# ColumbiaDVMM/ColumbiaImageSearch

Measured on AMD Instinct MI355X. Metric: queries/sec @ recall@10 on 10M LOPQ index, higher is better.
Workload: dtype f64

## Files before the change

### columbiaimagesearch_amd/csrc/lopq_scan3.hip

```cpp
#include "scan_common.h"
#include <cmath>
#include <cstdio>
#include <cstdlib>

typedef unsigned short u16x2_t __attribute__((ext_vector_type(2)));

static __device__ __forceinline__ uint32_t pk_add_u16(uint32_t a, uint32_t b) {
    return __builtin_bit_cast(uint32_t, (u16x2_t)(__builtin_bit_cast(u16x2_t, a) + __builtin_bit_cast(u16x2_t, b)));
}
static __device__ __forceinline__ uint32_t pk_subsat_u16(uint32_t a, uint32_t b) {
    return __builtin_bit_cast(uint32_t, __builtin_elementwise_sub_sat(__builtin_bit_cast(u16x2_t, a), __builtin_bit_cast(u16x2_t, b)));
}

static __device__ __forceinline__ uint32_t pk_min_u16(uint32_t a, uint32_t b) {
    return __builtin_bit_cast(uint32_t, __builtin_elementwise_min(__builtin_bit_cast(u16x2_t, a), __builtin_bit_cast(u16x2_t, b)));
}

static const int S3G = 4;

#ifdef CIS_S3_COUNTERS
__device__ unsigned long long g_s3_ctr[16];
#define S3_CLK() ((long long)__builtin_amdgcn_s_memtime())
#define S3_CTR(i, v) do { if (threadIdx.x == 0) atomicAdd(&g_s3_ctr[i], (unsigned long long)(v)); } while (0)
extern "C" int cis_debug_counters3(unsigned long long* out, int reset) {
// ... 140 lines not shown
    for (int r = 0; r < NR; ++r) {
        const bool kp = keep[r] && s[r] <= cut;
        const unsigned long long m = __ballot(kp);
        const int idx = ncnt + __builtin_amdgcn_mbcnt_hi((unsigned)(m >> 32), __builtin_amdgcn_mbcnt_lo((unsigned)m, 0));
        if (kp) rk[idx] = ent[r];
        ncnt += __popcll(m);
    }
    __builtin_amdgcn_fence(__ATOMIC_RELEASE, "wavefront");
    __builtin_amdgcn_wave_barrier();
    return ncnt;
}

template <int M, int NR, int NW>
__device__ __forceinline__ int wave_compact3_exact(uint32_t* rk, int cnt, int L, int Lw, const QScale& qs, Scan3Shared* sh, int w,
                                                   const uint8_t* __restrict__ codes, int64_t start, int K,
                                                   const double* __restrict__ t0, const double* __restrict__ t1, uint32_t& dup_pos) {
    const int lane = threadIdx.x & 63;
    const uint64_t INF64 = 0x7ff0000000000000ull;
    uint32_t hi[NR], lo[NR], ent[NR];
    bool keep[NR];
    uint32_t mn = 0xffffffffu, mx = 0u;
#pragma unroll
    for (int r = 0; r < NR; ++r) {
        const int e = r * 64 + lane;
        keep[r] = e < cnt;
        ent[r] = keep[r] ? rk[e] : 0xffffffffu;
        hi[r] = 0xffffffffu;
        lo[r] = 0xffffffffu;
    }
#pragma unroll
    for (int r = 0; r < NR; ++r) {
        if (r * 64 >= cnt) break;
        const CodeWords<M> cw = load_code<M>(codes, start + (keep[r] ? (ent[r] & 0xffffu) : 0u));
        const uint64_t k = keep[r] ? (uint64_t)__double_as_longlong(adc64_words<M>(cw.w, K, t0, t1)) : ~0ull;
        hi[r] = (uint32_t)(k >> 32);
        lo[r] = (uint32_t)k;
        mn = (keep[r] && hi[r] < mn) ? hi[r] : mn;
        mx = (keep[r] && hi[r] > mx) ? hi[r] : mx;
    }
    wave_minmax_step<1>(mn, mx); wave_minmax_step<2>(mn, mx); wave_minmax_step<4>(mn, mx);
    wave_minmax_step<8>(mn, mx); wave_minmax_step<16>(mn, mx); wave_minmax_step<32>(mn, mx);
    mn = (uint32_t)__builtin_amdgcn_readfirstlane((int)mn);
    mx = (uint32_t)__builtin_amdgcn_readfirstlane((int)mx);
    uint32_t vhiL = mx;
    uint64_t boundL = INF64;
    if (cnt >= L) {
        const uint32_t vhi = wave_kth_bisect<NR>(hi, keep, mn, mx, L);
        vhiL = vhi;
        boundL = hi_to_bound(vhi);
        int c_less = 0, g = 0;
#pragma unroll
        for (int r = 0; r < NR; ++r) {
            c_less += __popcll(__ballot(keep[r] && hi[r] < vhi));
// ... 125 lines not shown
    for (int i = 1; i < OCT; ++i) {
        a0 = pk_add_u16(a0, f[i][0]);
        a1 = pk_add_u16(a1, f[i][1]);
    }
    u32x2_t r;
    r[0] = a0; r[1] = a1;
    return r;
}

static __device__ __forceinline__ uint32_t ld16(const uint16_t* p) { return *reinterpret_cast<const volatile uint16_t*>(p); }
static __device__ __forceinline__ void st16(uint16_t* p, uint32_t v) { *reinterpret_cast<volatile uint16_t*>(p) = (uint16_t)v; }

template <int M, int NR, int U, int NW>
__device__ __forceinline__ void scan3_group(const WorkItem* __restrict__ items, const TabDesc* __restrict__ tabs,
                                            const int (&item_idx)[S3G], int ng,
                                            const double* __restrict__ T, const float* __restrict__ T32,
                                            const uint8_t* __restrict__ codes, int K, int L, int S,
                                            uint64_t* __restrict__ item_surv, int* __restrict__ item_n, float* __restrict__ item_slack,
                                            unsigned long long* __restrict__ qbound, char* smem, bool two_pass) {
    constexpr int G = S3G;
    constexpr int R = NR * 64 - 8;
    constexpr int nf = M / 2;
    constexpr int OCT = M >= 8 ? 8 : 4, NU = M / OCT;
    constexpr uint32_t CAP = 65535u / M;
    char* tab = smem;
    uint32_t* rk_all = reinterpret_cast<uint32_t*>(smem + (size_t)K * M * G * 2);
    Scan3Shared* sh = reinterpret_cast<Scan3Shared*>(rk_all + G * NW * R);
    uint16_t* thr1 = reinterpret_cast<uint16_t*>(sh + G);
    const int tid = threadIdx.x, lane = tid & 63;
    const int w = __builtin_amdgcn_readfirstlane(tid >> 6);
    const long long c0 = S3_CLK();
// ... 418 lines not shown
                        u0 = u;
                        continue;
                    }
                    const int idx = cnt[g] + __builtin_amdgcn_mbcnt_hi((unsigned)(m >> 32), __builtin_amdgcn_mbcnt_lo((unsigned)m, 0));
                    if ((m >> lane) & 1ull) rk[idx] = entry(u);
                    cnt[g] += n;
                    u0 = u + 1;
                }
                if (!full) break;
                const QScale qsg = load_scale(&sh[g]);
                int c2 = wave_compact3<M, NR, NW>(rk, cnt[g], L, Lw, R - 64, qsg, &sh[g], w);
                if (c2 < 0) {
                    uint32_t dp = 0xffffffffu;
                    const WorkItem itg = items[item_idx[g]];
                    c2 = wave_compact3_exact<M, NR, NW>(rk, cnt[g], L, Lw, qsg, &sh[g], w, codes, start, K,
                                                        T + (int64_t)itg.tab0 * nf * K, T + (int64_t)itg.tab1 * nf * K, dp);
                    dp = (uint32_t)__builtin_amdgcn_readfirstlane((int)dp);
                    if (dp != 0xffffffffu) {
                        dup[g] = load_code<M>(codes, start + (int64_t)dp);
                        has_dup[g] = true;
                        any_dup = true;
                    }
                }
                cnt[g] = c2;
                const uint32_t thg = lds_ld(&sh[g].thr);
                if (lane == 0) st16(&thr1[g], thg + 1u);
                const unsigned long long dup_on = has_dup[g] ? ~0ull : 0ull;
#pragma unroll
                for (int u = 0; u < U; ++u) {
                    const uint32_t sg = (g & 1) ? (d[u][g >> 1] >> 16) : (d[u][g >> 1] & 0xffffu);
                    bool same = true;
// ... 40 lines not shown
        }
        uint64_t* out = item_surv + (int64_t)item_idx[g] * S + off;
        for (int e = lane; e < cnt[g]; e += 64) {
            const uint32_t x = rk[e];
            out[e] = ((uint64_t)(x >> 16) << 32) | (x & 0xffffu);
        }
        if (tid == 0) item_n[item_idx[g]] = total;
    }
    S3_CTR(7, S3_CLK() - c0);
    S3_CTR(0, 1);
}

template <int M, int NR, int U, int NW, int WPE>
__global__ __launch_bounds__(NW * 64) __attribute__((amdgpu_waves_per_eu(WPE, WPE))) void k_adc_scan3(
    const WorkItem* __restrict__ items, const TabDesc* __restrict__ tabs, const int* __restrict__ slots,
    const int* __restrict__ n_slots_ptr, const double* __restrict__ T, const float* __restrict__ T32,
    const uint8_t* __restrict__ codes, int K, int L, int S, int* __restrict__ queue_ctr ,
    uint64_t* __restrict__ item_surv, int* __restrict__ item_n, float* __restrict__ item_slack,
    unsigned long long* __restrict__ qbound , int two_pass, int single_queue ) {
    extern __shared__ __attribute__((aligned(16))) char smem[];
    constexpr int G = S3G;
    constexpr int R = NR * 64 - 8;
    int* s_next = reinterpret_cast<int*>(smem + (size_t)K * M * G * 2 + (size_t)G * NW * R * 4 + G * sizeof(Scan3Shared) + 32);
    const int* qs = n_slots_ptr + 8;
    const int home = blockIdx.x & 7;
    const long long k0 = S3_CLK();
    (void)k0;
    for (int a = 0; a < 8; ++a) {
        const int x = (home + a) & 7;
        const int qstart = qs[x];
        const int count = single_queue ? (x == 0 ? qs[1] - qstart : 0) : qs[x + 1] - qstart;
// ... 27 lines not shown
                } else {
                    idx[g] = idx[0];
                }
            }
            if (!same) {
                for (int g2 = 0; g2 < ng; ++g2) {
                    int oi[G];
#pragma unroll
                    for (int g = 0; g < G; ++g) {
                        oi[g] = idx[0];
#pragma unroll
                        for (int gg = 1; gg < G; ++gg)
                            if (gg == g2) oi[g] = idx[gg];
                    }
                    if (g2 > 0) __syncthreads();
                    scan3_group<M, NR, U, NW>(items, tabs, oi, 1, T, T32, codes, K, L, S, item_surv, item_n, item_slack, qbound, smem, two_pass != 0);
                }
                continue;
            }
            scan3_group<M, NR, U, NW>(items, tabs, idx, ng, T, T32, codes, K, L, S, item_surv, item_n, item_slack, qbound, smem, two_pass != 0);
        }
    }
    S3_CTR(9, S3_CLK() - k0);
    S3_CTR(10, 1);
}

struct Slot4 {
    int item[S3G], tab0[S3G], tab1[S3G], q[S3G];
    float qinv[S3G];
    int start_lo, start_hi, len, ng;
    int ist_lo[S3G], ist_hi[S3G], ilen[S3G];
};
struct Scan4Shared {
    double inv_up, ub;
    uint64_t ext;
// ... 1294 lines not shown
                       S5_B, nsamp, ss_env, hits, hitn, slack, cnt_ok, ovf);
    hipLaunchKernelGGL(k_scan5_tau<S5_B / 64>, dim3((unsigned)((nq + 3) / 4)), dim3(256), 0, st, bmin, S5_B, nsamp, plan, nq, P, tau);
    if (ev_main) (void)hipEventRecord(ev_main, st);
    hipLaunchKernelGGL((k_adc_scan5<M, false, WPE>), dim3(grid), dim3(256), lds, st, items, tabs, slots, n_slots, T32, T, codes, K, g.S, tau, bmin, S5_B, nsamp,
                       ss_env, hits, hitn, slack, cnt_ok, ovf);
    const int64_t max_slots = n_items + 8;
    hipLaunchKernelGGL(k_scan5_check, dim3((unsigned)((max_slots + 255) / 256)), dim3(256), 0, st, slots, n_slots, items, plan, cnt_ok, ovf, L, fhdr, fslots, hitn,
                       qctr + 9);
    if (getenv("CIS_SCAN5_DEBUG")) {
        int h[6] = {0, 0, 0, 0, 0, 0};
        if (hipMemcpyAsync(h, qctr + 9, sizeof(h), hipMemcpyDeviceToHost, st) == hipSuccess && hipStreamSynchronize(st) == hipSuccess)
            fprintf(stderr, "[cis] k_adc_scan5: %d slots to the fall-back list\n", h[1]);
    }
    constexpr int U = 4, NW = 4;
    constexpr int WPE3 = 4;
    hipLaunchKernelGGL((k_adc_scan3<M, NR, U, NW, WPE3>), dim3(256), dim3(NW * 64), g.lds, st, items, tabs, fslots, fhdr + 8, T, T32, codes, K, L, g.S, fhdr, hits, hitn,
                       slack, qbound, g.long_chunks ? 0 : 1, 1);
}

void launch_scan5(int M, const Scan3Geom& g, int64_t n_items, int nq, hipStream_t st, const WorkItem* items, const TabDesc* tabs, const int* slots,
                  const int* n_slots, const PlanOut* plan, const double* T, const float* T32, const uint8_t* codes, int K, int L, int* qctr, uint64_t* hits,
                  int* hitn, float* slack, unsigned long long* qbound, int* fhdr, int* fslots, void* ws, hipEvent_t ev_main) {
    if (M == 4) {
        if (L <= 184) launch_scan5_t<4, 4>(g, n_items, nq, st, items, tabs, slots, n_slots, plan, T, T32, codes, K, L, qctr, hits, hitn, slack, qbound, fhdr, fslots, ws, ev_main);
        else launch_scan5_t<4, 8>(g, n_items, nq, st, items, tabs, slots, n_slots, plan, T, T32, codes, K, L, qctr, hits, hitn, slack, qbound, fhdr, fslots, ws, ev_main);
    } else {
        if (L <= 184) launch_scan5_t<8, 4>(g, n_items, nq, st, items, tabs, slots, n_slots, plan, T, T32, codes, K, L, qctr, hits, hitn, slack, qbound, fhdr, fslots, ws, ev_main);
        else launch_scan5_t<8, 8>(g, n_items, nq, st, items, tabs, slots, n_slots, plan, T, T32, codes, K, L, qctr, hits, hitn, slack, qbound, fhdr, fslots, ws, ev_main);
    }
}

bool scan3_supported(int M, int K, int L) {
// ... 12 lines not shown
    g.long_chunks = avg_chunk >= 6144 ? 1 : 0;
    static const int s4_m16 = getenv("CIS_S4_M16") ? atoi(getenv("CIS_S4_M16")) : 1;
    if (g.two_pass == 0 && g.long_chunks && (M <= 8 || s4_m16) && L <= 128) g.two_pass = 2;
    if (const char* e = getenv("CIS_SCAN3_TWOPASS")) g.two_pass = atoi(e);
    if (force_two_pass >= 0) g.two_pass = force_two_pass;
    if (g.two_pass == 2 && M > 8 && !s4_m16 && force_two_pass != 2) g.two_pass = g.long_chunks ? 0 : 1;
    if (g.two_pass == 1 && g.long_chunks && force_two_pass < 0) g.two_pass = 0;
    if (g.two_pass < 0 || g.two_pass > 2) g.two_pass = 0;
    g.S = g.NW * (NR * 64 - 8);
    g.lds = (size_t)K * M * g.G * 2 + (size_t)g.G * g.NW * (NR * 64 - 8) * 4 + g.G * sizeof(Scan3Shared) + 32 + 16;
    return g;
}

template <int M, int NR, int NW>
static void launch_scan3_t(const Scan3Geom& g, int64_t n_items, hipStream_t st, const WorkItem* items, const TabDesc* tabs,
                           const int* slots, const int* n_slots, const double* T, const float* T32, const uint8_t* codes, int K,
                           int L, int* qctr, uint64_t* hits, int* hitn, float* slack, unsigned long long* qbound, int* fhdr, int* fslots) {
    constexpr int U = 4;
    constexpr int WPE = M == 16 ? (NW == 4 ? 3 : 2) : (NW == 4 ? 4 : (NW == 2 ? 3 : 2));
    const int by_lds = (int)(163840 / g.lds), by_waves = (WPE * 4) / NW;
    const int per_cu = by_lds < by_waves ? by_lds : by_waves;
    const int64_t resident = 256 * (per_cu < 1 ? 1 : per_cu);
    const int64_t want = (n_items + g.G - 1) / g.G + 8;
    const unsigned grid = (unsigned)(want < resident ? ((want + 7) / 8) * 8 : resident);
    if constexpr (NW == 4) {
        if (g.two_pass == 2) {
            const float z_short = getenv("CIS_S4_ZS") ? (float)atof(getenv("CIS_S4_ZS")) : CIS_S4_Z;
            const float z_long = getenv("CIS_S4_ZL") ? (float)atof(getenv("CIS_S4_ZL")) : 4.5f;
            const int frac_long = getenv("CIS_S4_FRAC") ? atoi(getenv("CIS_S4_FRAC")) : 8;
            const int nsx_long = getenv("CIS_S4_NSX") ? atoi(getenv("CIS_S4_NSX")) : 128;
            const int dyn_long = getenv("CIS_S4_DYN") ? atoi(getenv("CIS_S4_DYN")) : 0;
// ... 25 lines not shown
                    const size_t lds4 = scan4_lds(M, K, S4_LCAP_LONG, 8);
                    hipLaunchKernelGGL((k_adc_scan4<M, CIS_S4_UL, 8, WPE8, S4_LCAP_LONG>), dim3(grid_of(lds4, WPE8, 8)), dim3(8 * 64), lds4, st, items, tabs, slots,
                                       n_slots, T32, T, codes, K, L, g.S, dbg4, fhdr, fslots, hits, hitn, slack, qbound, z_long, frac_long, nsx_long, dyn_long, g.sat);
                } else {
                    const size_t lds4 = scan4_lds(M, K, S4_LCAP_LONG, NW);
                    hipLaunchKernelGGL((k_adc_scan4<M, CIS_S4_UL, NW, WPE4, S4_LCAP_LONG>), dim3(grid_of(lds4, WPE4, NW)), dim3(NW * 64), lds4, st, items, tabs, slots,
                                       n_slots, T32, T, codes, K, L, g.S, dbg4, fhdr, fslots, hits, hitn, slack, qbound, z_long, frac_long, nsx_long, dyn_long, g.sat);
                }
            }
            if (getenv("CIS_SCAN4_DEBUG")) {
                int h[6] = {0, 0, 0, 0, 0, 0};
                if (hipMemcpyAsync(h, qctr + 9, sizeof(h), hipMemcpyDeviceToHost, st) == hipSuccess && hipStreamSynchronize(st) == hipSuccess)
                    fprintf(stderr, "[cis] k_adc_scan4: %d slots, %d to the fall-back list (lists: %d overflowed, %d failed the verification, %d crowds at the cut; %d slots with items of different chunks)\n",
                            h[0], h[1], h[2], h[3], h[4], h[5]);
            }
            hipLaunchKernelGGL((k_adc_scan3<M, NR, U, NW, WPE>), dim3(256), dim3(NW * 64), g.lds, st, items, tabs, fslots, fhdr + 8, T, T32,
                               codes, K, L, g.S, fhdr, hits, hitn, slack, qbound, g.long_chunks ? 0 : 1, 1);
            return;
        }
    }
    hipLaunchKernelGGL((k_adc_scan3<M, NR, U, NW, WPE>), dim3(grid), dim3(NW * 64), g.lds, st, items, tabs, slots, n_slots, T, T32,
                       codes, K, L, g.S, qctr, hits, hitn, slack, qbound, g.two_pass, 0);
}

void launch_scan3(int M, const Scan3Geom& g, int64_t n_items, hipStream_t st, const WorkItem* items, const TabDesc* tabs,
                  const int* slots, const int* n_slots, const double* T, const float* T32, const uint8_t* codes, int K, int L,
                  int* qctr, uint64_t* hits, int* hitn, float* slack, unsigned long long* qbound, int* fhdr, int* fslots) {
#define CIS_S3_NW(MM, RR) launch_scan3_t<MM, RR, 4>(g, n_items, st, items, tabs, slots, n_slots, T, T32, codes, K, L, qctr, hits, hitn, slack, qbound, fhdr, fslots)
#define CIS_S3(MM)                   \
    do {                             \
        if (L <= 184) CIS_S3_NW(MM, 4); \
        else CIS_S3_NW(MM, 8);       \
    } while (0)
    if (M == 4) CIS_S3(4);
    else if (M == 8) CIS_S3(8);
    else CIS_S3(16);
#undef CIS_S3
#undef CIS_S3_NW
}
```

### columbiaimagesearch_amd/csrc/lopq_search.hip

```cpp
#include <atomic>
#include <chrono>
#include <mutex>
#include <algorithm>

#include "lopq_index.h"
#include "scan_common.h"


static __device__ __forceinline__ uint64_t f2bits(double d) { return (uint64_t)__double_as_longlong(d); }
static __device__ __forceinline__ uint64_t f2bits(float f) { return (uint64_t)__float_as_uint(f); }

static const int GRP_SUB = 32;
#define GRP_WORDS(V) (6 * (V) * GRP_SUB + 2)
#define GRP_TILES(V) ((2 * (V) * GRP_SUB + 1023) / 1024)

template <typename CT>
__global__ void k_rank(const CT* __restrict__ dist , int nq, int V,
                       uint16_t* __restrict__ order , CT* __restrict__ sorted ,
                       int* __restrict__ grp ) {
    extern __shared__ __attribute__((aligned(16))) char smem[];
    uint64_t* sb = reinterpret_cast<uint64_t*>(smem);
    const int q = blockIdx.x, s = blockIdx.y;
    if (q == 0 && s == 0)
        for (int i = threadIdx.x; i < 4 * V * GRP_SUB; i += blockDim.x) grp[i] = 0;
// ... 1309 lines not shown
#endif
    if (threadIdx.x < nt) ssplit[threadIdx.x] = tabs[t0 + threadIdx.x].split;
    __syncthreads();
    const bool on = k < K;
    double sc[W];
    const double* src = subs + ((int64_t)(z * nf + j) * K + (on ? k : 0)) * W;
#pragma unroll
    for (int i = 0; i < W; ++i) sc[i] = src[i];
    for (int t = 0; t < nt; ++t) {
        if (ssplit[t] != z) continue;
#ifndef CIS_TABLES_SCALAR_PX
        const double* f = sf[t];
#else
        const double* f = px + (int64_t)(t0 + t) * h + j * W;
#endif
        auto elem = [&](int i) -> double { const double df = f[i] - sc[i]; return df * df; };
        const double v = pw_leaf<double>(elem, 0, W);
        const float v32 = (float)v;
        if (on) {
#ifndef CIS_TABLES_NO_NT
            __builtin_nontemporal_store(v, &T[((int64_t)(t0 + t) * nf + j) * K + k]);
#else
            T[((int64_t)(t0 + t) * nf + j) * K + k] = v;
#endif
            if (T32) T32[((int64_t)(t0 + t) * nf + j) * K + k] = v32;
        }
        uint32_t b = on ? __float_as_uint(v32) : 0u, dummy = 0u;
        wave_minmax_step<1>(dummy, b); wave_minmax_step<2>(dummy, b); wave_minmax_step<4>(dummy, b);
        wave_minmax_step<8>(dummy, b); wave_minmax_step<16>(dummy, b); wave_minmax_step<32>(dummy, b);
        if ((threadIdx.x & 63) == 0) atomicMax(reinterpret_cast<unsigned int*>(&tabs[t0 + t].pad), b);
    }
}

__global__ void k_tables_f32(const double* __restrict__ T, int64_t n, int nf, int K, float* __restrict__ T32, TabDesc* __restrict__ tabs) {
    const int64_t e = (int64_t)blockIdx.x * blockDim.x + threadIdx.x;
    if (e >= n) return;
    const float v = (float)T[e];
    T32[e] = v;
// ... 1188 lines not shown
                if (gt == asc) { ka[i] = a1; kb[i] = b1; ka[p] = a0; kb[p] = b0; }
            }
            wave_lds_sync();
        }
    }
}

template <int CAPM, int MT , int NEMAX >
#ifndef CIS_MERGE_WPE
#define CIS_MERGE_WPE 4
#endif
__global__ __launch_bounds__(256) __attribute__((amdgpu_waves_per_eu((MT == 16 || MT == 0) ? 2 : CIS_MERGE_WPE, 8)))
void k_merge_survivors(const uint64_t* __restrict__ surv ,
                                                         const int* __restrict__ item_n, const int64_t* __restrict__ item_off,
                                                         const WorkItem* __restrict__ items, const double* __restrict__ T,
                                                         const uint8_t* __restrict__ codes, const int64_t* __restrict__ ids,
                                                         int nq, int M, int K, int limit, int S,
                                                         cis_hit* __restrict__ out_hits, int64_t* __restrict__ out_ids,
                                                         double* __restrict__ out_dists, int* __restrict__ out_n,
                                                         int32_t* __restrict__ out_cells, uint32_t* __restrict__ out_pos,
                                                         const PlanOut* __restrict__ plan, int32_t* __restrict__ out_visited,
                                                         const float* __restrict__ item_slack ) {
    extern __shared__ __attribute__((aligned(16))) char smem[];
    const int lane = threadIdx.x & 63, wq = threadIdx.x >> 6;
    const int q = blockIdx.x * 4 + wq;
    if (q >= nq) return;
    if (lane == 0 && out_visited) out_visited[q] = plan[q].visited;
    uint64_t* ka = reinterpret_cast<uint64_t*>(smem) + (size_t)wq * 2 * CAPM;
    uint64_t* kb = ka + CAPM;
    const int64_t first = item_off[q];
// ... 69 lines not shown
                if (item_slack) {
                    const float s_i = li[i] == 0 ? sl[0] : (li[i] == 1 ? sl[1] : (li[i] == 2 ? sl[2] : sl[3]));
                    keep[i] = valid[i] && ((double)__uint_as_float(hi[i]) - (double)s_i <= (double)vub);
                }
                const unsigned long long m = __ballot(keep[i]);
                idx[i] = kept + __builtin_amdgcn_mbcnt_hi((unsigned)(m >> 32), __builtin_amdgcn_mbcnt_lo((unsigned)m, 0));
                kept += __popcll(m);
            }
            if (kept > CAPM) return false;
            WorkItem its[4];
#pragma unroll
            for (int i = 0; i < 4; ++i) its[i] = items[first + (i < n_lists ? i : 0)];
#pragma unroll
            for (int i0 = 0; i0 < NE; i0 += 4) {
                int64_t startv[4];
                const double* t0v[4];
                const double* t1v[4];
                uint32_t rankv[4], pos0v[4];
#pragma unroll
                for (int i = 0; i < 4; ++i) {
                    WorkItem it = its[0];
#pragma unroll
                    for (int j = 1; j < 4; ++j)
                        if (li[i0 + i] == j) it = its[j];
                    startv[i] = it.start; rankv[i] = (uint32_t)it.rank; pos0v[i] = (uint32_t)it.pos0;
                    t0v[i] = T + (int64_t)it.tab0 * nf * K;
                    t1v[i] = T + (int64_t)it.tab1 * nf * K;
                }
                CodeWords<MT> cw[4];
#pragma unroll
                for (int i = 0; i < 4; ++i) cw[i] = load_code<MT>(codes, startv[i] + (keep[i0 + i] ? pp[i0 + i] : 0u));
                double dd[4];
#pragma unroll
                for (int i = 0; i < 4; ++i) dd[i] = adc64_words<MT>(cw[i].w, K, t0v[i], t1v[i]);
#pragma unroll
                for (int i = 0; i < 4; ++i) {
                    if (keep[i0 + i]) {
                        ka[idx[i0 + i]] = (uint64_t)__double_as_longlong(dd[i]);
                        kb[idx[i0 + i]] = ((uint64_t)rankv[i] << 32) | (uint32_t)(pos0v[i] + pp[i0 + i]);
                    }
                }
            }
            int ns = 64;
            while (ns < kept) ns <<= 1;
            for (int x = kept + lane; x < ns; x += 64) { ka[x] = ~0ull; kb[x] = ~0ull; }
            wave_lds_sync();
            wave_bitonic_lds(ka, kb, ns);
            total = kept;
            return true;
// ... 24 lines not shown
                    }
                } else {
                    for (int x0 = 0; x0 < take; x0 += 256) {
                        uint32_t p[4];
                        bool on[4];
#pragma unroll
                        for (int i = 0; i < 4; ++i) {
                            const int x = x0 + i * 64 + lane;
                            on[i] = x < take;
                            p[i] = on[i] ? (uint32_t)src[x] : 0u;
                        }
                        CodeWords<MT> cw[4];
#pragma unroll
                        for (int i = 0; i < 4; ++i) cw[i] = load_code<MT>(codes, it.start + p[i]);
                        double dd[4];
#pragma unroll
                        for (int i = 0; i < 4; ++i) dd[i] = adc64_words<MT>(cw[i].w, K, t0, t1);
#pragma unroll
                        for (int i = 0; i < 4; ++i) {
                            const int x = x0 + i * 64 + lane;
                            if (on[i]) {
                                ka[n + x] = (uint64_t)__double_as_longlong(dd[i]);
                                kb[n + x] = ((uint64_t)(uint32_t)it.rank << 32) | (uint32_t)(it.pos0 + (int)p[i]);
                            }
                        }
                    }
                }
            }
            n += take;
            total += take;
            room -= take;
            e += take;
// ... 1850 lines not shown
    TabDesc* tabs = ix->w_tabs.as<TabDesc>();
    CIS_TRY(ix->w_tord.reserve((size_t)(n_tabs + 1) * sizeof(int)));
    int* tab_order = ix->w_tord.as<int>();
    double* T = ix->w_T.as<double>();
    static const bool no_t32 = getenv("CIS_NO_T32") != nullptr && atoi(getenv("CIS_NO_T32")) != 0;
    const bool drop_t32 = no_t32 && !direct_elig && (m->w == 4 || m->w == 8 || m->w == 16 || m->w == 32) && K <= 256;
    if (!drop_t32) CIS_TRY(ix->w_T32.reserve(direct_elig ? (size_t)(n_tabs + 1) * h * sizeof(float) : (size_t)(n_tabs + 1) * nf * K * sizeof(float)));
    float* T32 = drop_t32 ? nullptr : ix->w_T32.as<float>();
    const size_t tab_lds = (size_t)(2 * h + (h < 256 ? 256 : 0)) * sizeof(double);
    const bool split_tables = (m->w == 4 || m->w == 8 || m->w == 16 || m->w == 32) && K <= 256;
    double* px_buf = nullptr;
    if (split_tables) {
        CIS_TRY(ix->w_px.reserve((size_t)(n_tabs + 1) * h * sizeof(double)));
        px_buf = ix->w_px.as<double>();
    }
    if (ct == CIS_F32) {
        if (par_plan)
            hipLaunchKernelGGL((k_plan_par<float, true>), dim3(nq), dim3(256), 0, st, ix->w_sorted.as<float>(), ix->w_order.as<uint16_t>(),
                               ix->gcount_ptr(), ix->loff_ptr(), nq, V, quota, seg_max, plan, item_off, tab_off, items,
                               tabs, nullptr, grp_base, grp_cur, tab_order, vis_list, plan_fb, vis_cap, nullptr, 0);
        hipLaunchKernelGGL((k_plan<float, true>), dim3(nq), dim3(64), plan_lds, st, ix->w_sorted.as<float>(),
                           ix->w_order.as<uint16_t>(), ix->gcount_ptr(), ix->loff_ptr(), nq, V, quota,
                           seg_max, plan, item_off, tab_off, items, tabs, nullptr, grp_base, grp_cur, tab_order, plan_fb);
        if (n_tabs > 0)
            launch_tables<float>(n_tabs, tab_lds, st, (const float*)xc, m->d_Cs32, m->d_Rt, m->d_mus, m->d_subs, tabs, tab_order, V, h,
                                 m->w, nf, K, D, T, m->prog_w, px_buf, d_tot, direct_elig ? T32 : nullptr);
    } else {
        if (par_plan)
            hipLaunchKernelGGL((k_plan_par<double, true>), dim3(nq), dim3(256), 0, st, ix->w_sorted.as<double>(), ix->w_order.as<uint16_t>(),
                               ix->gcount_ptr(), ix->loff_ptr(), nq, V, quota, seg_max, plan, item_off, tab_off, items,
                               tabs, nullptr, grp_base, grp_cur, tab_order, vis_list, plan_fb, vis_cap, nullptr, 0);
        hipLaunchKernelGGL((k_plan<double, true>), dim3(nq), dim3(64), plan_lds, st, ix->w_sorted.as<double>(),
                           ix->w_order.as<uint16_t>(), ix->gcount_ptr(), ix->loff_ptr(), nq, V, quota,
                           seg_max, plan, item_off, tab_off, items, tabs, nullptr, grp_base, grp_cur, tab_order, plan_fb);
        if (n_tabs > 0)
            launch_tables<double>(n_tabs, tab_lds, st, (const double*)xc, m->d_Cs64, m->d_Rt, m->d_mus, m->d_subs, tabs, tab_order, V,
                                  h, m->w, nf, K, D, T, m->prog_w, px_buf, d_tot, direct_elig ? T32 : nullptr);
    }
    const bool direct = direct_elig;
    if (direct) {
    } else if (split_tables && n_tabs > 0) {
        const bool few = n_tabs <= 1024;
        dim3 g((unsigned)ceil_div(n_tabs, few ? 8 : 64), (unsigned)nf, 2);
#define CIS_TFP(WW)                                                                                                                                      \
        if (few) hipLaunchKernelGGL((k_tables_from_px<WW, 8>), g, dim3(256), 0, st, px_buf, tabs, (int)n_tabs, m->d_subs, h, nf, K, T, T32, d_tot);      \
        else hipLaunchKernelGGL((k_tables_from_px<WW, 64>), g, dim3(256), 0, st, px_buf, tabs, (int)n_tabs, m->d_subs, h, nf, K, T, T32, d_tot)
        switch (m->w) {
            case 4: CIS_TFP(4); break;
            case 8: CIS_TFP(8); break;
            case 16: CIS_TFP(16); break;
            default: CIS_TFP(32); break;
        }
#undef CIS_TFP
    } else if (fast && n_tabs > 0) {
        const int64_t ne = n_tabs * nf * K;
        hipLaunchKernelGGL(k_tables_f32, dim3((unsigned)ceil_div(ne, 256)), dim3(256), 0, st, T, ne, nf, K, T32, tabs);
    }
    if (stream) {
        CIS_TRY(mark(2));
        const uint8_t* codes = ix->codes_ptr();
        const int64_t* ids = ix->ids_ptr();
// ... 219 lines not shown
            hipLaunchKernelGGL(k_copy_visited, dim3((unsigned)ceil_div(nq, 256)), dim3(256), 0, st, plan, nq, out.visited);
        CIS_CHECK_HIP(hipGetLastError());
        CIS_TRY(mark(4));
        if (ix->profiling) ix->prof.push_back(pr);
        return CIS_OK;
    }
    CIS_TRY(mark(2));
    if (n_items > 0) {
        pr.has_scan = true;
        const uint8_t* codes = ix->codes_ptr();
        const int64_t* ids = ix->ids_ptr();
        cis_hit* hits = ix->w_hits.as<cis_hit>();
        int* hitn = ix->w_hitn.as<int>();
        if (fast) {
            const bool sort_items = ix->ncells <= 65536;
            static const int env_s5 = getenv("CIS_SCAN5") ? atoi(getenv("CIS_SCAN5")) : 0;
            const bool use5 = use3 && geom3.two_pass == 2 && scan5_supported(M, K, L) && (ix->force_scan5 || (env_s5 != 0 && !ix->force_scan3 && L <= 128));
            const int G = use5 ? 8 : (use3 ? geom3.G : geom.G);
            int64_t CH = use3 ? ceil_div(ix->max_cell > 0 ? ix->max_cell : 1, (int64_t)seg_max) : 1;
            CH = CH < 1 ? 1 : (CH > 16 ? 16 : CH);
            const int64_t nkeys = 2 * ix->ncells * CH;
            const int64_t max_slots = sort_items ? (n_items + nkeys) / G + nkeys + 2 : n_items;
            CIS_TRY(ix->w_order2.reserve((size_t)(64 + 2 * nkeys + 2 * max_slots * G) * sizeof(int)));
            int* qctr = ix->w_order2.as<int>();
            int* n_slots = qctr + 8;
            int* qstart = qctr + 16;
            int* fhdr = qctr + 32;
            int* cell_cnt = qctr + 64;
            int* slot_off = cell_cnt + nkeys;
            int* slots = slot_off + nkeys;
            int* fslots = slots + max_slots * G;
            if (sort_items) {
// ... 9 lines not shown
                CIS_CHECK_HIP(hipMemsetAsync(qctr, 0, 64 * sizeof(int), st));
                hipLaunchKernelGGL(k_identity_slots, dim3((unsigned)ceil_div(n_items < 9 ? 9 : n_items, 256)), dim3(256), 0, st, n_items, G,
                                   slots, n_slots, qstart);
            }
            CIS_TRY(mark(5));
            ix->last_scan_kernel = use5 ? 6 : (use3 ? (geom3.two_pass == 2 ? 4 : 3) : 2);
            if (use5) {
                CIS_TRY(ix->w_s5.reserve(scan5_workspace_bytes(nq)));
                launch_scan5(M, geom3, n_items, nq, st, items, tabs, slots, n_slots, plan, T, T32, codes, K, L, qctr, ix->w_hits.as<uint64_t>(), hitn,
                             ix->w_slack.as<float>(), qbound, fhdr, fslots, ix->w_s5.p, nullptr);
            } else
            if (use3) {
                Scan3Geom g3 = geom3;
                const float sat16 = getenv("CIS_S4_SAT") ? (float)atof(getenv("CIS_S4_SAT")) : 0.75f;
                if (M == 16 && g3.two_pass == 2) g3.sat = sat16;
                launch_scan3(M, g3, n_items, st, items, tabs, slots, n_slots, T, T32, codes, K, L, qctr, ix->w_hits.as<uint64_t>(), hitn, ix->w_slack.as<float>(), qbound, fhdr, fslots);
                if (g3.sat > 0.f && ix->h_totals)
                    CIS_CHECK_HIP(hipMemcpyAsync(&ix->h_totals[4], qctr + 9, 2 * sizeof(int), hipMemcpyDeviceToHost, st));
            }
            else
                launch_scan2(M, geom, n_items, st, items, slots, n_slots, T, T32, codes, ids, K, L, qctr, ix->w_hits.as<uint64_t>(), hitn, qbound);
        }
        else {
            CIS_TRY(mark(5));
            ix->last_scan_kernel = 1;
            launch_scan_exact(M, n_items, st, items, T, codes, ids, K, L, S, nullptr, hits, hitn);
        }
        ix->stats[3] += 1;
    }
    CIS_TRY(mark(3));
    {
        const cis_hit* hits = ix->w_hits.as<cis_hit>();
        const int* hitn = ix->w_hitn.as<int>();
        if (fast) {
            const uint64_t* surv = ix->w_hits.as<uint64_t>();
            const uint8_t* codes = ix->codes_ptr();
            const int64_t* ids = ix->ids_ptr();
            const bool many = n_items > nq + nq / 4;
#define CIS_MERGE_SURV(CAP, MT)                                                                                              \
    do {                                                                                                                     \
        if (many)                                                                                                            \
            hipLaunchKernelGGL((k_merge_survivors<CAP, MT, 8>), dim3((unsigned)ceil_div(nq, 4)), dim3(256), (size_t)4 * CAP * 16, st, \
                               surv, hitn, item_off, items, T, codes, ids, nq, M, K, L, S, out.hits, out.ids, out.dists,     \
                               out.n_found, out.cells, out.pos, plan, out.visited, use3 ? ix->w_slack.as<float>() : (const float*)nullptr);                            \
        else                                                                                                                 \
            hipLaunchKernelGGL((k_merge_survivors<CAP, MT, 4>), dim3((unsigned)ceil_div(nq, 4)), dim3(256), (size_t)4 * CAP * 16, st, \
                               surv, hitn, item_off, items, T, codes, ids, nq, M, K, L, S, out.hits, out.ids, out.dists,     \
                               out.n_found, out.cells, out.pos, plan, out.visited, use3 ? ix->w_slack.as<float>() : (const float*)nullptr);                            \
    } while (0)
#define CIS_MERGE_SURV_M(CAP)                                                                          \
    do {                                                                                               \
        if (M == 4) CIS_MERGE_SURV(CAP, 4); else if (M == 8) CIS_MERGE_SURV(CAP, 8); else CIS_MERGE_SURV(CAP, 16); \
    } while (0)
            if (L <= 128) CIS_MERGE_SURV_M(256);
            else if (L <= 256) CIS_MERGE_SURV_M(512);
            else if (L <= 440) CIS_MERGE_SURV_M(1024);
            else CIS_MERGE_SURV_M(2048);
#undef CIS_MERGE_SURV_M
#undef CIS_MERGE_SURV
        } else if (L <= 512)
            hipLaunchKernelGGL(k_merge_items<1024>, dim3(nq), dim3(256), (size_t)1024 * 24 + 16, st, hits, hitn, item_off, L, S, out.hits,
                               out.ids, out.dists, out.n_found, out.cells, out.pos);
// ... 813 lines not shown
```

### columbiaimagesearch_amd/csrc/scan_common.h

```cpp
#pragma once
#include "lopq_model.h"

struct WorkItem {
    int q;
    int rank;
    int tab0, tab1;
    int64_t start;
    int len;
    int pos0;
    int cell;
    int pad;
};

struct TabDesc {
    int q, split, cluster, pad;
};

struct PlanOut {
    int visited, n_items, ntab0, ntab1;
    int64_t ncand;
};

template <int LJ>
__device__ __forceinline__ uint32_t lane_xor(uint32_t v) {
// ... 129 lines not shown
template <int M>
__device__ __forceinline__ CodeWords<M> load_code(const uint8_t* __restrict__ codes, int64_t p) {
    CodeWords<M> c;
    if constexpr (M == 4) {
        c.w[0] = *reinterpret_cast<const uint32_t*>(codes + p * 4);
    } else if constexpr (M == 8) {
        const uint2 v = *reinterpret_cast<const uint2*>(codes + p * 8);
        c.w[0] = v.x; c.w[1] = v.y;
    } else {
        const uint4 v = *reinterpret_cast<const uint4*>(codes + p * 16);
        c.w[0] = v.x; c.w[1] = v.y; c.w[2] = v.z; c.w[3] = v.w;
    }
    return c;
}

template <int M>
struct RotConsts {
    uint32_t sh[4];
    uint32_t cj[M];
    uint32_t hsel;
};

template <int M>
__device__ __forceinline__ RotConsts<M> make_rot(int lane) {
    RotConsts<M> rc;
    const int r = lane & (M - 1);
    const int h = r >> 2, q = r & 3;
    rc.hsel = (uint32_t)h;
#pragma unroll
    for (int tq = 0; tq < 4; ++tq) rc.sh[tq] = 8u * (uint32_t)((q + tq) & 3);
// ... 32 lines not shown
    if (T32) return reinterpret_cast<const float4*>(T32 + tab * nfK)[e4];
    const double2* p = reinterpret_cast<const double2*>(T + tab * nfK) + 2 * e4;
    const double2 a = p[0], b = p[1];
    return make_float4((float)a.x, (float)a.y, (float)b.x, (float)b.y);
}
static __device__ __forceinline__ float tab_f1(const float* __restrict__ T32, const double* __restrict__ T, int64_t idx) {
    return T32 ? T32[idx] : (float)T[idx];
}

struct Scan3Geom { int G, NW, U, S, two_pass, long_chunks; size_t lds;
                   float sat = 0.f; };
bool scan3_supported(int M, int K, int L);
Scan3Geom scan3_geom(int M, int K, int L, int64_t avg_chunk ,
                     int force_two_pass );
void launch_scan3(int M, const Scan3Geom& g, int64_t n_items, hipStream_t st, const WorkItem* items, const TabDesc* tabs,
                  const int* slots, const int* n_slots, const double* T, const float* T32, const uint8_t* codes, int K, int L,
                  int* qctr, uint64_t* hits, int* hitn, float* slack, unsigned long long* qbound,
                  int* fhdr , int* fslots );

static const int STREAM_B = 4096;
static const int STREAM_CAP = 16384;
bool stream_supported(int M, int K, int L);
int stream_grid(int M, int G, int K, int64_t max_rows);
int stream_max_group();
size_t stream_slot_bytes();
void launch_stream_prep(hipStream_t st, const WorkItem* items, int64_t n_items, const int64_t* item_off, int nq, int64_t n_cand,
                        const int* slots , int* n_slots, int G, int M, int64_t* cand_start, int64_t* seg,
                        unsigned long long* qmin, unsigned long long* qmax, int* cnt, int* status, int64_t* rowoff ,
                        void* desc , const int64_t* d_totals );
void launch_stream_scan(int M, int G, bool sample, int grid, hipStream_t st, const void* desc, const int* n_slots, const int64_t* rowoff,
                        const float* T32, const double* T, const uint8_t* codes, int K, const float* tau,
// ... 16 lines not shown
```

Before: 22.70 million.

## Compute exact f64 ADC distances on demand instead of materializing f64 tables

When the fast scan3 path with f32 tables is in use, the f64 distance table is no longer written. The exact rescoring in wave_compact3_exact and k_merge_survivors instead recomputes each sub-distance from the residual projections and the sub-codebook rows. This removes the f64 table store traffic and its memory footprint. In exchange, survivors and compaction fallbacks pay extra loads and arithmetic per code (W-wide rows for M subquantizers).

```diff
diff --git a/columbiaimagesearch_amd/csrc/lopq_scan3.hip b/columbiaimagesearch_amd/csrc/lopq_scan3.hip
--- a/columbiaimagesearch_amd/csrc/lopq_scan3.hip
+++ b/columbiaimagesearch_amd/csrc/lopq_scan3.hip
@@ -178,7 +178,8 @@
 template <int M, int NR, int NW>
 __device__ __forceinline__ int wave_compact3_exact(uint32_t* rk, int cnt, int L, int Lw, const QScale& qs, Scan3Shared* sh, int w,
                                                    const uint8_t* __restrict__ codes, int64_t start, int K,
-                                                   const double* __restrict__ t0, const double* __restrict__ t1, uint32_t& dup_pos) {
+                                                   const double* __restrict__ t0, const double* __restrict__ t1, const Tab64Src& src,
+                                                   int tab0, int tab1, uint32_t& dup_pos) {
     const int lane = threadIdx.x & 63;
     const uint64_t INF64 = 0x7ff0000000000000ull;
     uint32_t hi[NR], lo[NR], ent[NR];
@@ -192,6 +193,26 @@
         hi[r] = 0xffffffffu;
         lo[r] = 0xffffffffu;
     }
+    if (src.px) {
+#pragma unroll 1
+        for (int r0 = 0; r0 * 64 < cnt; ++r0) {
+            const bool kp = r0 * 64 + lane < cnt;
+            const CodeWords<M> cw[1] = {load_code<M>(codes, start + (kp ? (rk[r0 * 64 + lane] & 0xffffu) : 0u))};
+            const int ta[1] = {tab0}, tb[1] = {tab1};
+            double dd[1];
+            adc64_words_src<M, 1>(src, cw, K, ta, tb, dd);
+            const uint64_t k = kp ? (uint64_t)__double_as_longlong(dd[0]) : ~0ull;
+#pragma unroll
+            for (int r = 0; r < NR; ++r) {
+                if (r == r0) {
+                    hi[r] = (uint32_t)(k >> 32);
+                    lo[r] = (uint32_t)k;
+                }
+            }
+            mn = (kp && (uint32_t)(k >> 32) < mn) ? (uint32_t)(k >> 32) : mn;
+            mx = (kp && (uint32_t)(k >> 32) > mx) ? (uint32_t)(k >> 32) : mx;
+        }
+    } else {
 #pragma unroll
     for (int r = 0; r < NR; ++r) {
         if (r * 64 >= cnt) break;
@@ -201,6 +222,7 @@
         lo[r] = (uint32_t)k;
         mn = (keep[r] && hi[r] < mn) ? hi[r] : mn;
         mx = (keep[r] && hi[r] > mx) ? hi[r] : mx;
+    }
     }
     wave_minmax_step<1>(mn, mx); wave_minmax_step<2>(mn, mx); wave_minmax_step<4>(mn, mx);
     wave_minmax_step<8>(mn, mx); wave_minmax_step<16>(mn, mx); wave_minmax_step<32>(mn, mx);
@@ -356,7 +378,7 @@
 template <int M, int NR, int U, int NW>
 __device__ __forceinline__ void scan3_group(const WorkItem* __restrict__ items, const TabDesc* __restrict__ tabs,
                                             const int (&item_idx)[S3G], int ng,
-                                            const double* __restrict__ T, const float* __restrict__ T32,
+                                            const double* __restrict__ T, const Tab64Src& src, const float* __restrict__ T32,
                                             const uint8_t* __restrict__ codes, int K, int L, int S,
                                             uint64_t* __restrict__ item_surv, int* __restrict__ item_n, float* __restrict__ item_slack,
                                             unsigned long long* __restrict__ qbound, char* smem, bool two_pass) {
@@ -805,7 +827,7 @@
                     uint32_t dp = 0xffffffffu;
                     const WorkItem itg = items[item_idx[g]];
                     c2 = wave_compact3_exact<M, NR, NW>(rk, cnt[g], L, Lw, qsg, &sh[g], w, codes, start, K,
-                                                        T + (int64_t)itg.tab0 * nf * K, T + (int64_t)itg.tab1 * nf * K, dp);
+                                                        T + (int64_t)itg.tab0 * nf * K, T + (int64_t)itg.tab1 * nf * K, src, itg.tab0, itg.tab1, dp);
                     dp = (uint32_t)__builtin_amdgcn_readfirstlane((int)dp);
                     if (dp != 0xffffffffu) {
                         dup[g] = load_code<M>(codes, start + (int64_t)dp);
@@ -876,7 +898,8 @@
 template <int M, int NR, int U, int NW, int WPE>
 __global__ __launch_bounds__(NW * 64) __attribute__((amdgpu_waves_per_eu(WPE, WPE))) void k_adc_scan3(
     const WorkItem* __restrict__ items, const TabDesc* __restrict__ tabs, const int* __restrict__ slots,
-    const int* __restrict__ n_slots_ptr, const double* __restrict__ T, const float* __restrict__ T32,
+    const int* __restrict__ n_slots_ptr, const double* __restrict__ T, const Tab64Src src ,
+    const float* __restrict__ T32,
     const uint8_t* __restrict__ codes, int K, int L, int S, int* __restrict__ queue_ctr ,
     uint64_t* __restrict__ item_surv, int* __restrict__ item_n, float* __restrict__ item_slack,
     unsigned long long* __restrict__ qbound , int two_pass, int single_queue ) {
@@ -934,11 +957,11 @@
                             if (gg == g2) oi[g] = idx[gg];
                     }
                     if (g2 > 0) __syncthreads();
-                    scan3_group<M, NR, U, NW>(items, tabs, oi, 1, T, T32, codes, K, L, S, item_surv, item_n, item_slack, qbound, smem, two_pass != 0);
+                    scan3_group<M, NR, U, NW>(items, tabs, oi, 1, T, src, T32, codes, K, L, S, item_surv, item_n, item_slack, qbound, smem, two_pass != 0);
                 }
                 continue;
             }
-            scan3_group<M, NR, U, NW>(items, tabs, idx, ng, T, T32, codes, K, L, S, item_surv, item_n, item_slack, qbound, smem, two_pass != 0);
+            scan3_group<M, NR, U, NW>(items, tabs, idx, ng, T, src, T32, codes, K, L, S, item_surv, item_n, item_slack, qbound, smem, two_pass != 0);
         }
     }
     S3_CTR(9, S3_CLK() - k0);
@@ -2263,8 +2286,8 @@
     }
     constexpr int U = 4, NW = 4;
     constexpr int WPE3 = 4;
-    hipLaunchKernelGGL((k_adc_scan3<M, NR, U, NW, WPE3>), dim3(256), dim3(NW * 64), g.lds, st, items, tabs, fslots, fhdr + 8, T, T32, codes, K, L, g.S, fhdr, hits, hitn,
-                       slack, qbound, g.long_chunks ? 0 : 1, 1);
+    hipLaunchKernelGGL((k_adc_scan3<M, NR, U, NW, WPE3>), dim3(256), dim3(NW * 64), g.lds, st, items, tabs, fslots, fhdr + 8, T, Tab64Src{nullptr, nullptr, 0, 0} ,
+                       T32, codes, K, L, g.S, fhdr, hits, hitn, slack, qbound, g.long_chunks ? 0 : 1, 1);
 }
 
 void launch_scan5(int M, const Scan3Geom& g, int64_t n_items, int nq, hipStream_t st, const WorkItem* items, const TabDesc* tabs, const int* slots,
@@ -2307,7 +2330,7 @@
 
 template <int M, int NR, int NW>
 static void launch_scan3_t(const Scan3Geom& g, int64_t n_items, hipStream_t st, const WorkItem* items, const TabDesc* tabs,
-                           const int* slots, const int* n_slots, const double* T, const float* T32, const uint8_t* codes, int K,
+                           const int* slots, const int* n_slots, const double* T, const Tab64Src& src, const float* T32, const uint8_t* codes, int K,
                            int L, int* qctr, uint64_t* hits, int* hitn, float* slack, unsigned long long* qbound, int* fhdr, int* fslots) {
     constexpr int U = 4;
     constexpr int WPE = M == 16 ? (NW == 4 ? 3 : 2) : (NW == 4 ? 4 : (NW == 2 ? 3 : 2));
@@ -2363,19 +2386,19 @@
                     fprintf(stderr, "[cis] k_adc_scan4: %d slots, %d to the fall-back list (lists: %d overflowed, %d failed the verification, %d crowds at the cut; %d slots with items of different chunks)\n",
                             h[0], h[1], h[2], h[3], h[4], h[5]);
             }
-            hipLaunchKernelGGL((k_adc_scan3<M, NR, U, NW, WPE>), dim3(256), dim3(NW * 64), g.lds, st, items, tabs, fslots, fhdr + 8, T, T32,
+            hipLaunchKernelGGL((k_adc_scan3<M, NR, U, NW, WPE>), dim3(256), dim3(NW * 64), g.lds, st, items, tabs, fslots, fhdr + 8, T, src, T32,
                                codes, K, L, g.S, fhdr, hits, hitn, slack, qbound, g.long_chunks ? 0 : 1, 1);
             return;
         }
     }
-    hipLaunchKernelGGL((k_adc_scan3<M, NR, U, NW, WPE>), dim3(grid), dim3(NW * 64), g.lds, st, items, tabs, slots, n_slots, T, T32,
+    hipLaunchKernelGGL((k_adc_scan3<M, NR, U, NW, WPE>), dim3(grid), dim3(NW * 64), g.lds, st, items, tabs, slots, n_slots, T, src, T32,
                        codes, K, L, g.S, qctr, hits, hitn, slack, qbound, g.two_pass, 0);
 }
 
 void launch_scan3(int M, const Scan3Geom& g, int64_t n_items, hipStream_t st, const WorkItem* items, const TabDesc* tabs,
-                  const int* slots, const int* n_slots, const double* T, const float* T32, const uint8_t* codes, int K, int L,
+                  const int* slots, const int* n_slots, const double* T, const Tab64Src& src, const float* T32, const uint8_t* codes, int K, int L,
                   int* qctr, uint64_t* hits, int* hitn, float* slack, unsigned long long* qbound, int* fhdr, int* fslots) {
-#define CIS_S3_NW(MM, RR) launch_scan3_t<MM, RR, 4>(g, n_items, st, items, tabs, slots, n_slots, T, T32, codes, K, L, qctr, hits, hitn, slack, qbound, fhdr, fslots)
+#define CIS_S3_NW(MM, RR) launch_scan3_t<MM, RR, 4>(g, n_items, st, items, tabs, slots, n_slots, T, src, T32, codes, K, L, qctr, hits, hitn, slack, qbound, fhdr, fslots)
 #define CIS_S3(MM)                   \
     do {                             \
         if (L <= 184) CIS_S3_NW(MM, 4); \
diff --git a/columbiaimagesearch_amd/csrc/lopq_search.hip b/columbiaimagesearch_amd/csrc/lopq_search.hip
--- a/columbiaimagesearch_amd/csrc/lopq_search.hip
+++ b/columbiaimagesearch_amd/csrc/lopq_search.hip
@@ -1347,14 +1347,13 @@
 #else
         const double* f = px + (int64_t)(t0 + t) * h + j * W;
 #endif
-        auto elem = [&](int i) -> double { const double df = f[i] - sc[i]; return df * df; };
-        const double v = pw_leaf<double>(elem, 0, W);
+        const double v = tab_entry64<W>(f, sc);
         const float v32 = (float)v;
         if (on) {
 #ifndef CIS_TABLES_NO_NT
-            __builtin_nontemporal_store(v, &T[((int64_t)(t0 + t) * nf + j) * K + k]);
+            if (T) __builtin_nontemporal_store(v, &T[((int64_t)(t0 + t) * nf + j) * K + k]);
 #else
-            T[((int64_t)(t0 + t) * nf + j) * K + k] = v;
+            if (T) T[((int64_t)(t0 + t) * nf + j) * K + k] = v;
 #endif
             if (T32) T32[((int64_t)(t0 + t) * nf + j) * K + k] = v32;
         }
@@ -2573,6 +2572,7 @@
 void k_merge_survivors(const uint64_t* __restrict__ surv ,
                                                          const int* __restrict__ item_n, const int64_t* __restrict__ item_off,
                                                          const WorkItem* __restrict__ items, const double* __restrict__ T,
+                                                         const Tab64Src tsrc ,
                                                          const uint8_t* __restrict__ codes, const int64_t* __restrict__ ids,
                                                          int nq, int M, int K, int limit, int S,
                                                          cis_hit* __restrict__ out_hits, int64_t* __restrict__ out_ids,
@@ -2672,8 +2672,7 @@
 #pragma unroll
             for (int i0 = 0; i0 < NE; i0 += 4) {
                 int64_t startv[4];
-                const double* t0v[4];
-                const double* t1v[4];
+                int tab0v[4], tab1v[4];
                 uint32_t rankv[4], pos0v[4];
 #pragma unroll
                 for (int i = 0; i < 4; ++i) {
@@ -2682,15 +2681,19 @@
                     for (int j = 1; j < 4; ++j)
                         if (li[i0 + i] == j) it = its[j];
                     startv[i] = it.start; rankv[i] = (uint32_t)it.rank; pos0v[i] = (uint32_t)it.pos0;
-                    t0v[i] = T + (int64_t)it.tab0 * nf * K;
-                    t1v[i] = T + (int64_t)it.tab1 * nf * K;
+                    tab0v[i] = it.tab0; tab1v[i] = it.tab1;
                 }
                 CodeWords<MT> cw[4];
 #pragma unroll
                 for (int i = 0; i < 4; ++i) cw[i] = load_code<MT>(codes, startv[i] + (keep[i0 + i] ? pp[i0 + i] : 0u));
                 double dd[4];
-#pragma unroll
-                for (int i = 0; i < 4; ++i) dd[i] = adc64_words<MT>(cw[i].w, K, t0v[i], t1v[i]);
+                if (tsrc.px) {
+                    adc64_words_src<MT, 4>(tsrc, cw, K, tab0v, tab1v, dd);
+                } else {
+#pragma unroll
+                    for (int i = 0; i < 4; ++i)
+                        dd[i] = adc64_words<MT>(cw[i].w, K, T + (int64_t)tab0v[i] * nf * K, T + (int64_t)tab1v[i] * nf * K);
+                }
 #pragma unroll
                 for (int i = 0; i < 4; ++i) {
                     if (keep[i0 + i]) {
@@ -2745,8 +2748,13 @@
 #pragma unroll
                         for (int i = 0; i < 4; ++i) cw[i] = load_code<MT>(codes, it.start + p[i]);
                         double dd[4];
-#pragma unroll
-                        for (int i = 0; i < 4; ++i) dd[i] = adc64_words<MT>(cw[i].w, K, t0, t1);
+                        if (tsrc.px) {
+                            const int tab0v[4] = {it.tab0, it.tab0, it.tab0, it.tab0}, tab1v[4] = {it.tab1, it.tab1, it.tab1, it.tab1};
+                            adc64_words_src<MT, 4>(tsrc, cw, K, tab0v, tab1v, dd);
+                        } else {
+#pragma unroll
+                            for (int i = 0; i < 4; ++i) dd[i] = adc64_words<MT>(cw[i].w, K, t0, t1);
+                        }
 #pragma unroll
                         for (int i = 0; i < 4; ++i) {
                             const int x = x0 + i * 64 + lane;
@@ -4627,6 +4635,13 @@
         CIS_TRY(ix->w_px.reserve((size_t)(n_tabs + 1) * h * sizeof(double)));
         px_buf = ix->w_px.as<double>();
     }
+    static const int env_s5 = getenv("CIS_SCAN5") ? atoi(getenv("CIS_SCAN5")) : 0;
+    const bool use5 = use3 && geom3.two_pass == 2 && scan5_supported(M, K, L) && (ix->force_scan5 || (env_s5 != 0 && !ix->force_scan3 && L <= 128));
+    const char* env_f64 = getenv("CIS_TABLES_F64");
+    const bool on_demand = fast && use3 && !use5 && split_tables && !direct_elig && !stream && !big && !ix->stream_off && T32 != nullptr &&
+                           (M == 4 || M == 8 || M == 16) && !(env_f64 && atoi(env_f64) != 0);
+    const Tab64Src src64 = {on_demand ? px_buf : nullptr, m->d_subs, h, m->w};
+    double* T_out = on_demand ? nullptr : T;
     if (ct == CIS_F32) {
         if (par_plan)
             hipLaunchKernelGGL((k_plan_par<float, true>), dim3(nq), dim3(256), 0, st, ix->w_sorted.as<float>(), ix->w_order.as<uint16_t>(),
@@ -4656,8 +4671,8 @@
         const bool few = n_tabs <= 1024;
         dim3 g((unsigned)ceil_div(n_tabs, few ? 8 : 64), (unsigned)nf, 2);
 #define CIS_TFP(WW)                                                                                                                                      \
-        if (few) hipLaunchKernelGGL((k_tables_from_px<WW, 8>), g, dim3(256), 0, st, px_buf, tabs, (int)n_tabs, m->d_subs, h, nf, K, T, T32, d_tot);      \
-        else hipLaunchKernelGGL((k_tables_from_px<WW, 64>), g, dim3(256), 0, st, px_buf, tabs, (int)n_tabs, m->d_subs, h, nf, K, T, T32, d_tot)
+        if (few) hipLaunchKernelGGL((k_tables_from_px<WW, 8>), g, dim3(256), 0, st, px_buf, tabs, (int)n_tabs, m->d_subs, h, nf, K, T_out, T32, d_tot);  \
+        else hipLaunchKernelGGL((k_tables_from_px<WW, 64>), g, dim3(256), 0, st, px_buf, tabs, (int)n_tabs, m->d_subs, h, nf, K, T_out, T32, d_tot)
         switch (m->w) {
             case 4: CIS_TFP(4); break;
             case 8: CIS_TFP(8); break;
@@ -4907,8 +4922,6 @@
         int* hitn = ix->w_hitn.as<int>();
         if (fast) {
             const bool sort_items = ix->ncells <= 65536;
-            static const int env_s5 = getenv("CIS_SCAN5") ? atoi(getenv("CIS_SCAN5")) : 0;
-            const bool use5 = use3 && geom3.two_pass == 2 && scan5_supported(M, K, L) && (ix->force_scan5 || (env_s5 != 0 && !ix->force_scan3 && L <= 128));
             const int G = use5 ? 8 : (use3 ? geom3.G : geom.G);
             int64_t CH = use3 ? ceil_div(ix->max_cell > 0 ? ix->max_cell : 1, (int64_t)seg_max) : 1;
             CH = CH < 1 ? 1 : (CH > 16 ? 16 : CH);
@@ -4948,7 +4961,7 @@
                 Scan3Geom g3 = geom3;
                 const float sat16 = getenv("CIS_S4_SAT") ? (float)atof(getenv("CIS_S4_SAT")) : 0.75f;
                 if (M == 16 && g3.two_pass == 2) g3.sat = sat16;
-                launch_scan3(M, g3, n_items, st, items, tabs, slots, n_slots, T, T32, codes, K, L, qctr, ix->w_hits.as<uint64_t>(), hitn, ix->w_slack.as<float>(), qbound, fhdr, fslots);
+                launch_scan3(M, g3, n_items, st, items, tabs, slots, n_slots, T, src64, T32, codes, K, L, qctr, ix->w_hits.as<uint64_t>(), hitn, ix->w_slack.as<float>(), qbound, fhdr, fslots);
                 if (g3.sat > 0.f && ix->h_totals)
                     CIS_CHECK_HIP(hipMemcpyAsync(&ix->h_totals[4], qctr + 9, 2 * sizeof(int), hipMemcpyDeviceToHost, st));
             }
@@ -4975,11 +4988,11 @@
     do {                                                                                                                     \
         if (many)                                                                                                            \
             hipLaunchKernelGGL((k_merge_survivors<CAP, MT, 8>), dim3((unsigned)ceil_div(nq, 4)), dim3(256), (size_t)4 * CAP * 16, st, \
-                               surv, hitn, item_off, items, T, codes, ids, nq, M, K, L, S, out.hits, out.ids, out.dists,     \
+                               surv, hitn, item_off, items, T, src64, codes, ids, nq, M, K, L, S, out.hits, out.ids, out.dists, \
                                out.n_found, out.cells, out.pos, plan, out.visited, use3 ? ix->w_slack.as<float>() : (const float*)nullptr);                            \
         else                                                                                                                 \
             hipLaunchKernelGGL((k_merge_survivors<CAP, MT, 4>), dim3((unsigned)ceil_div(nq, 4)), dim3(256), (size_t)4 * CAP * 16, st, \
-                               surv, hitn, item_off, items, T, codes, ids, nq, M, K, L, S, out.hits, out.ids, out.dists,     \
+                               surv, hitn, item_off, items, T, src64, codes, ids, nq, M, K, L, S, out.hits, out.ids, out.dists, \
                                out.n_found, out.cells, out.pos, plan, out.visited, use3 ? ix->w_slack.as<float>() : (const float*)nullptr);                            \
     } while (0)
 #define CIS_MERGE_SURV_M(CAP)                                                                          \
diff --git a/columbiaimagesearch_amd/csrc/scan_common.h b/columbiaimagesearch_amd/csrc/scan_common.h
--- a/columbiaimagesearch_amd/csrc/scan_common.h
+++ b/columbiaimagesearch_amd/csrc/scan_common.h
@@ -167,6 +167,89 @@
     return c;
 }
 
+template <class PF, class PS>
+static __device__ __forceinline__ double tab_entry64_n(const PF& f, const PS& sc, int n) {
+    auto elem = [&](int i) -> double { const double df = f[i] - sc[i]; return df * df; };
+    return pw_leaf<double>(elem, 0, n);
+}
+template <int W, class PF, class PS>
+static __device__ __forceinline__ double tab_entry64(const PF& f, const PS& sc) {
+    static_assert(W == 4 || W == 8 || W == 16 || W == 32, "tab_entry64: sub-vector width");
+    return tab_entry64_n(f, sc, W);
+}
+
+template <int W>
+static __device__ __forceinline__ void ld_row64(const double* __restrict__ p, double (&v)[W]) {
+#pragma unroll
+    for (int i = 0; i < W / 2; ++i) {
+        const double2 x = reinterpret_cast<const double2*>(p)[i];
+        v[2 * i] = x.x;
+        v[2 * i + 1] = x.y;
+    }
+}
+
+struct Tab64Src {
+    const double* px;
+    const double* subs;
+    int h, W;
+};
+
+template <int M, int W, int NC>
+static __device__ __forceinline__ void adc64_words_px(const CodeWords<M> (&cw)[NC], int K, const double* const (&f0)[NC],
+                                                      const double* const (&f1)[NC], const double* __restrict__ subs, double (&dd)[NC]) {
+    constexpr int nf = M / 2;
+#pragma unroll 1
+    for (int j = 0; j < M; ++j) {
+        double e[NC];
+#pragma unroll
+        for (int i = 0; i < NC; ++i) {
+            uint32_t ws = cw[i].w[0];
+#pragma unroll
+            for (int q = 1; q < (M + 3) / 4; ++q) ws = (j >> 2) == q ? cw[i].w[q] : ws;
+            const uint32_t c = (ws >> (8 * (j & 3))) & 255u;
+            double s[W], f[W];
+            ld_row64<W>(subs + ((int64_t)j * K + c) * W, s);
+            ld_row64<W>(j < nf ? f0[i] + j * W : f1[i] + (j - nf) * W, f);
+            e[i] = tab_entry64<W>(f, s);
+        }
+#pragma unroll
+        for (int i = 0; i < NC; ++i) dd[i] = j == 0 ? e[i] : dd[i] + e[i];
+    }
+}
+
+template <int M, int NC>
+static __device__ __forceinline__ void adc64_words_src(const Tab64Src& src, const CodeWords<M> (&cw)[NC], int K, const int (&tab0)[NC],
+                                                       const int (&tab1)[NC], double (&dd)[NC]) {
+    const double* f0[NC];
+    const double* f1[NC];
+#pragma unroll
+    for (int i = 0; i < NC; ++i) {
+        f0[i] = src.px + (int64_t)tab0[i] * src.h;
+        f1[i] = src.px + (int64_t)tab1[i] * src.h;
+    }
+    auto part = [&](auto w_tag, auto n_tag) {
+        constexpr int W = decltype(w_tag)::value, NP = decltype(n_tag)::value < NC ? decltype(n_tag)::value : NC;
+#pragma unroll
+        for (int i0 = 0; i0 < NC; i0 += NP) {
+            CodeWords<M> c[NP];
+            const double* a0[NP];
+            const double* a1[NP];
+            double d[NP];
+#pragma unroll
+            for (int i = 0; i < NP; ++i) { c[i] = cw[i0 + i]; a0[i] = f0[i0 + i]; a1[i] = f1[i0 + i]; }
+            adc64_words_px<M, W, NP>(c, K, a0, a1, src.subs, d);
+#pragma unroll
+            for (int i = 0; i < NP; ++i) dd[i0 + i] = d[i];
+        }
+    };
+    switch (src.W) {
+        case 4: part(std::integral_constant<int, 4>(), std::integral_constant<int, 4>()); break;
+        case 8: part(std::integral_constant<int, 8>(), std::integral_constant<int, 4>()); break;
+        case 16: part(std::integral_constant<int, 16>(), std::integral_constant<int, 2>()); break;
+        default: part(std::integral_constant<int, 32>(), std::integral_constant<int, 1>()); break;
+    }
+}
+
 template <int M>
 struct RotConsts {
     uint32_t sh[4];
@@ -229,7 +312,8 @@
 Scan3Geom scan3_geom(int M, int K, int L, int64_t avg_chunk ,
                      int force_two_pass );
 void launch_scan3(int M, const Scan3Geom& g, int64_t n_items, hipStream_t st, const WorkItem* items, const TabDesc* tabs,
-                  const int* slots, const int* n_slots, const double* T, const float* T32, const uint8_t* codes, int K, int L,
+                  const int* slots, const int* n_slots, const double* T, const Tab64Src& src ,
+                  const float* T32, const uint8_t* codes, int K, int L,
                   int* qctr, uint64_t* hits, int* hitn, float* slack, unsigned long long* qbound,
                   int* fhdr , int* fslots );
 
```

Result: slower. 16.86 million (-25.7%).
